# linuxing3/weekend-raytracer-wgpu

Measured on AMD Instinct MI355X. Metric: Msamples/sec (pixels x spp) at 1920x1080, 1000 spp, higher is better.
Workload: dtype f32; 1 GPU; BASELINE configs[2]: path-traced 3-sphere scene, checker-diffuse ground + glass + metal (src/main.rs:539-541), 1920x1080, 1000 spp, 8 bounces, gradient sky, seed 0; width=1920, height=1080, spp=1000, num_bounces=8, mode=pt, partition=whole frame

## Files before the change

include/mirt.h:

```cpp
#ifndef MIRT_H
#define MIRT_H

#include <stddef.h>
#include <stdint.h>

#ifdef __cplusplus
extern "C" {
#endif

#define MIRT_VERSION_MAJOR 0
#define MIRT_VERSION_MINOR 4
#define MIRT_VERSION_PATCH 0


typedef struct MirtSphere {
    float    center[4];
    float    radius;
    uint32_t material_idx;
    uint32_t _pad[2];
} MirtSphere;

typedef struct MirtTextureDescriptor {
    uint32_t width;
    uint32_t height;
// ... 134 lines not shown
typedef struct MirtContext MirtContext;


uint32_t    mirt_version(void);
const char* mirt_last_error(void);
const char* mirt_status_string(int status);

int mirt_validate_render_params(const MirtCamera* camera, const MirtSamplingParams* sampling,
                                uint32_t viewport_w, uint32_t viewport_h);

int mirt_camera_new(const MirtCamera* camera, uint32_t viewport_w, uint32_t viewport_h,
                    MirtGpuCamera* out);

int mirt_camera_from_fly_pose(const float position[3], float yaw_radians, float pitch_radians,
                              float vfov_degrees, float aperture, float focus_distance,
                              MirtCamera* out);

float mirt_degrees_to_radians(float degrees);
float mirt_radians_to_degrees(float radians);

uint32_t mirt_params_out_rows(const MirtParams* params);
uint32_t mirt_params_out_row_index(const MirtParams* params, uint32_t i);

typedef struct MirtGridPlan {
    float    cell_factor;
    uint32_t blob_bytes;
    uint32_t n_cells;
    uint32_t n_entries;
    uint32_t n_big;
    uint32_t pool_slots;
} MirtGridPlan;
int mirt_grid_plan(const MirtSphere* spheres, uint32_t n_spheres, uint64_t lds_bytes_per_block, MirtGridPlan* out);

int  mirt_ctx_create(int device, MirtContext** out);
void mirt_ctx_destroy(MirtContext* ctx);

int mirt_ctx_set_scene(MirtContext* ctx, const MirtScene* scene);
enum {
    MIRT_SCENE_HBM = 1u << 0
};
#define MIRT_SCENE_HBM_MAX_SPHERES (1u << 24)
#define MIRT_BVH_MAX_DEPTH  32
#define MIRT_BVH_MAX_LEAF   4
#define MIRT_BVH_MAX_ALWAYS 64
#define MIRT_BVH_BIG_RADII  4
int mirt_ctx_set_scene_ex(MirtContext* ctx, const MirtScene* scene, uint32_t flags);
typedef struct MirtBvhPlan {
    uint32_t n_nodes, n_leaves, n_leaf_spheres, n_always, max_depth, max_leaf;
    uint64_t device_bytes;
} MirtBvhPlan;
int mirt_bvh_plan(const MirtSphere* spheres, uint32_t n_spheres, MirtBvhPlan* out);

int mirt_ctx_set_camera(MirtContext* ctx, const MirtGpuCamera* camera);

int mirt_ctx_render(MirtContext* ctx, const MirtParams* params, uint8_t* out_rgba8, size_t out_len);

int mirt_ctx_render_device(MirtContext* ctx, const MirtParams* params, void* d_out_rgba8,
                           size_t out_len, void* hip_stream);

const char* mirt_ctx_last_kernel(const MirtContext* ctx);

int mirt_ctx_synchronize(MirtContext* ctx);
int mirt_ctx_frame_stream(MirtContext* ctx, uint32_t index, void** out_hip_stream);
int mirt_ctx_set_timing(MirtContext* ctx, int enabled);
int mirt_ctx_get_stats(MirtContext* ctx, MirtStats* out);

// ... 73 lines not shown
```

rust/mirt-sys/src/lib.rs:

```rust
#![allow(non_camel_case_types)]

use std::os::raw::{c_char, c_int, c_void};

#[repr(C)]
#[derive(Clone, Copy, Debug, Default)]
pub struct MirtSphere {
    pub center: [f32; 4],
    pub radius: f32,
    pub material_idx: u32,
    pub _pad: [u32; 2],
}

#[repr(C)]
#[derive(Clone, Copy, Debug, Default)]
pub struct MirtTextureDescriptor {
    pub width: u32,
    pub height: u32,
    pub offset: u32,
}

#[repr(C)]
#[derive(Clone, Copy, Debug, Default)]
pub struct MirtMaterial {
    pub id: u32,
// ... 171 lines not shown
pub struct MirtContext {
    _private: [u8; 0],
}

pub const MIRT_NODE_MAX_MEMBERS: u32 = 16;
pub const MIRT_NODE_RCCL: u32 = 1 << 0;

#[repr(C)]
pub struct MirtNode {
    _private: [u8; 0],
}

#[repr(C)]
#[derive(Clone, Copy, Debug, Default)]
pub struct MirtNodeStats {
    pub n_members: u32,
    pub transport: u32,
    pub gather_ms: f64,
    pub assemble_ms: f64,
}

extern "C" {
    pub fn mirt_version() -> u32;
    pub fn mirt_last_error() -> *const c_char;
    pub fn mirt_status_string(status: c_int) -> *const c_char;
    pub fn mirt_validate_render_params(camera: *const MirtCamera, sampling: *const MirtSamplingParams, viewport_w: u32, viewport_h: u32) -> c_int;
    pub fn mirt_camera_new(camera: *const MirtCamera, viewport_w: u32, viewport_h: u32, out: *mut MirtGpuCamera) -> c_int;
    pub fn mirt_camera_from_fly_pose(position: *const f32, yaw_radians: f32, pitch_radians: f32, vfov_degrees: f32, aperture: f32, focus_distance: f32, out: *mut MirtCamera) -> c_int;
    pub fn mirt_degrees_to_radians(degrees: f32) -> f32;
    pub fn mirt_radians_to_degrees(radians: f32) -> f32;
    pub fn mirt_params_out_rows(params: *const MirtParams) -> u32;
    pub fn mirt_params_out_row_index(params: *const MirtParams, i: u32) -> u32;
    pub fn mirt_grid_plan(spheres: *const MirtSphere, n_spheres: u32, lds_bytes_per_block: u64, out: *mut MirtGridPlan) -> c_int;
    pub fn mirt_ctx_create(device: c_int, out: *mut *mut MirtContext) -> c_int;
    pub fn mirt_ctx_destroy(ctx: *mut MirtContext);
    pub fn mirt_ctx_set_scene(ctx: *mut MirtContext, scene: *const MirtScene) -> c_int;
    pub fn mirt_ctx_set_scene_ex(ctx: *mut MirtContext, scene: *const MirtScene, flags: u32) -> c_int;
    pub fn mirt_bvh_plan(spheres: *const MirtSphere, n_spheres: u32, out: *mut MirtBvhPlan) -> c_int;
    pub fn mirt_ctx_set_camera(ctx: *mut MirtContext, camera: *const MirtGpuCamera) -> c_int;
    pub fn mirt_ctx_render(ctx: *mut MirtContext, params: *const MirtParams, out_rgba8: *mut u8, out_len: usize) -> c_int;
    pub fn mirt_ctx_render_device(ctx: *mut MirtContext, params: *const MirtParams, d_out_rgba8: *mut c_void, out_len: usize, hip_stream: *mut c_void) -> c_int;
    pub fn mirt_ctx_synchronize(ctx: *mut MirtContext) -> c_int;
    pub fn mirt_ctx_get_stats(ctx: *mut MirtContext, out: *mut MirtStats) -> c_int;
    pub fn mirt_ctx_frame_stream(ctx: *mut MirtContext, index: u32, out_hip_stream: *mut *mut c_void) -> c_int;
    pub fn mirt_ctx_set_timing(ctx: *mut MirtContext, enabled: c_int) -> c_int;
    pub fn mirt_ctx_last_kernel(ctx: *const MirtContext) -> *const c_char;
    pub fn mirt_ctx_accum_reset(ctx: *mut MirtContext, params: *const MirtParams) -> c_int;
    pub fn mirt_ctx_accum_add(ctx: *mut MirtContext, params: *const MirtParams, hip_stream: *mut c_void) -> c_int;
    pub fn mirt_ctx_accum_samples(ctx: *const MirtContext) -> u32;
    pub fn mirt_ctx_accum_resolve(ctx: *mut MirtContext, params: *const MirtParams, out_rgba8: *mut u8, out_len: usize) -> c_int;
    pub fn mirt_ctx_accum_read(ctx: *mut MirtContext, out_sums: *mut u64, out_len_u64: usize) -> c_int;
    pub fn mirt_ctx_accum_frame_device(ctx: *mut MirtContext, params: *const MirtParams, d_out_rgba8: *mut c_void, out_len: usize, hip_stream: *mut c_void) -> c_int;
    pub fn mirt_ctx_accum_frame(ctx: *mut MirtContext, params: *const MirtParams, out_rgba8: *mut u8, out_len: usize) -> c_int;
    pub fn mirt_ctx_selftest_math(ctx: *mut MirtContext, out_mismatches: *mut u64) -> c_int;
    pub fn mirt_render(scene: *const MirtScene, params: *const MirtParams, device: c_int, out_rgba8: *mut u8, out_len: usize) -> c_int;
    pub fn mirt_rgba8_to_rgb8(rgba: *const u8, n_pixels: usize, rgb: *mut u8) -> c_int;
    pub fn mirt_jpeg_info(data: *const u8, len: usize, width: *mut u32, height: *mut u32) -> c_int;
    pub fn mirt_jpeg_decode_rgb8(data: *const u8, len: usize, rgb: *mut u8, rgb_len: usize) -> c_int;
    pub fn mirt_rgb8_to_texels(rgb: *const u8, n_pixels: usize, texels: *mut f32) -> c_int;
    pub fn mirt_jpeg_last_error() -> *const c_char;
    pub fn mirt_ctx_deinterleave_device(ctx: *mut MirtContext, params: *const MirtParams, d_parts: *const c_void, part_stride: usize, d_out_rgba8: *mut c_void, out_len: usize, hip_stream: *mut c_void) -> c_int;
    pub fn mirt_node_create(devices: *const c_int, n: u32, flags: u32, out: *mut *mut MirtNode) -> c_int;
    pub fn mirt_node_destroy(node: *mut MirtNode);
    pub fn mirt_node_set_scene(node: *mut MirtNode, scene: *const MirtScene) -> c_int;
    pub fn mirt_node_set_scene_ex(node: *mut MirtNode, scene: *const MirtScene, flags: u32) -> c_int;
    pub fn mirt_node_set_camera(node: *mut MirtNode, camera: *const MirtGpuCamera) -> c_int;
// ... 11 lines not shown
```

weekend-raytracer-wgpu_amd/_abi.py:

```python
from __future__ import annotations

import ctypes as C

MIRT_MODE_PARITY = 0
MIRT_MODE_PT = 1
MIRT_MAX_SPP_PER_CALL = 1 << 24

MIRT_FLAG_SKY_HOSEK = 1 << 0
MIRT_FLAG_NO_TONEMAP = 1 << 1
MIRT_FLAG_NO_SRGB = 1 << 2
MIRT_FLAG_COUNT_WORK = 1 << 3
MIRT_FLAG_KERNEL_STRIP = 1 << 4
MIRT_FLAG_KERNEL_POOL = 1 << 5
MIRT_FLAG_NO_GRID = 1 << 6
MIRT_FLAG_COUNT_GRID = 1 << 7
MIRT_FLAG_FAST_MATH = 1 << 8
MIRT_FLAG_TEXEL_TILES = 1 << 9

MIRT_SCENE_HBM = 1 << 0
MIRT_SCENE_HBM_MAX_SPHERES = 1 << 24
MIRT_BVH_MAX_DEPTH = 32
MIRT_BVH_MAX_LEAF = 4
MIRT_BVH_MAX_ALWAYS = 64
MIRT_BVH_BIG_RADII = 4
# ... 108 lines not shown

    def as_dict(self) -> dict:
        return {"kernel_ms": self.kernel_ms, "kernel_ms_total": self.kernel_ms_total, "launches": self.launches,
                "samples": self.samples, "rays": self.rays,
                "sphere_tests": self.sphere_tests, "roots": self.roots, "hits": self.hits,
                "scatter": list(self.scatter), "sky_misses": self.sky_misses,
                "lane_iterations": self.lane_iterations, "wave_iterations": self.wave_iterations,
                "grid_cells": self.grid_cells, "grid_wave_cells": self.grid_wave_cells,
                "texel_fetches": list(self.texel_fetches), "texel_tile_hits": list(self.texel_tile_hits)}


class MirtNodeStats(C.Structure):
    _fields_ = [("n_members", C.c_uint32), ("transport", C.c_uint32), ("gather_ms", C.c_double), ("assemble_ms", C.c_double)]

    def as_dict(self) -> dict:
        return {"n_members": self.n_members, "transport": self.transport, "gather_ms": self.gather_ms,
                "assemble_ms": self.assemble_ms}


_P = C.POINTER
SYMBOLS = {
    "mirt_version": (C.c_uint32, []),
    "mirt_last_error": (C.c_char_p, []),
    "mirt_status_string": (C.c_char_p, [C.c_int]),
    "mirt_validate_render_params": (C.c_int, [_P(MirtCamera), _P(MirtSamplingParams), C.c_uint32, C.c_uint32]),
    "mirt_camera_new": (C.c_int, [_P(MirtCamera), C.c_uint32, C.c_uint32, _P(MirtGpuCamera)]),
    "mirt_camera_from_fly_pose": (C.c_int, [_P(C.c_float), C.c_float, C.c_float, C.c_float, C.c_float,
                                            C.c_float, _P(MirtCamera)]),
    "mirt_degrees_to_radians": (C.c_float, [C.c_float]),
    "mirt_radians_to_degrees": (C.c_float, [C.c_float]),
    "mirt_params_out_rows": (C.c_uint32, [_P(MirtParams)]),
    "mirt_params_out_row_index": (C.c_uint32, [_P(MirtParams), C.c_uint32]),
    "mirt_grid_plan": (C.c_int, [C.c_void_p, C.c_uint32, C.c_uint64, _P(MirtGridPlan)]),
    "mirt_ctx_create": (C.c_int, [C.c_int, _P(C.c_void_p)]),
    "mirt_ctx_destroy": (None, [C.c_void_p]),
    "mirt_ctx_set_scene": (C.c_int, [C.c_void_p, _P(MirtScene)]),
    "mirt_ctx_set_scene_ex": (C.c_int, [C.c_void_p, _P(MirtScene), C.c_uint32]),
    "mirt_bvh_plan": (C.c_int, [C.c_void_p, C.c_uint32, _P(MirtBvhPlan)]),
    "mirt_ctx_set_camera": (C.c_int, [C.c_void_p, _P(MirtGpuCamera)]),
    "mirt_ctx_render": (C.c_int, [C.c_void_p, _P(MirtParams), C.c_void_p, C.c_size_t]),
    "mirt_ctx_render_device": (C.c_int, [C.c_void_p, _P(MirtParams), C.c_void_p, C.c_size_t, C.c_void_p]),
    "mirt_ctx_last_kernel": (C.c_char_p, [C.c_void_p]),
    "mirt_ctx_synchronize": (C.c_int, [C.c_void_p]),
    "mirt_ctx_get_stats": (C.c_int, [C.c_void_p, _P(MirtStats)]),
    "mirt_ctx_accum_reset": (C.c_int, [C.c_void_p, _P(MirtParams)]),
    "mirt_ctx_accum_add": (C.c_int, [C.c_void_p, _P(MirtParams), C.c_void_p]),
    "mirt_ctx_accum_samples": (C.c_uint32, [C.c_void_p]),
    "mirt_ctx_accum_resolve": (C.c_int, [C.c_void_p, _P(MirtParams), C.c_void_p, C.c_size_t]),
    "mirt_ctx_accum_read": (C.c_int, [C.c_void_p, C.c_void_p, C.c_size_t]),
    "mirt_ctx_accum_frame_device": (C.c_int, [C.c_void_p, _P(MirtParams), C.c_void_p, C.c_size_t, C.c_void_p]),
    "mirt_ctx_accum_frame": (C.c_int, [C.c_void_p, _P(MirtParams), C.c_void_p, C.c_size_t]),
    "mirt_ctx_selftest_math": (C.c_int, [C.c_void_p, _P(C.c_uint64)]),
    "mirt_ctx_set_timing": (C.c_int, [C.c_void_p, C.c_int]),
    "mirt_ctx_frame_stream": (C.c_int, [C.c_void_p, C.c_uint32, C.POINTER(C.c_void_p)]),
    "mirt_render": (C.c_int, [_P(MirtScene), _P(MirtParams), C.c_int, C.c_void_p, C.c_size_t]),
    "mirt_rgba8_to_rgb8": (C.c_int, [C.c_void_p, C.c_size_t, C.c_void_p]),
    "mirt_jpeg_info": (C.c_int, [C.c_void_p, C.c_size_t, _P(C.c_uint32), _P(C.c_uint32)]),
    "mirt_jpeg_decode_rgb8": (C.c_int, [C.c_void_p, C.c_size_t, C.c_void_p, C.c_size_t]),
    "mirt_rgb8_to_texels": (C.c_int, [C.c_void_p, C.c_size_t, C.c_void_p]),
    "mirt_jpeg_last_error": (C.c_char_p, []),
    "mirt_ctx_deinterleave_device": (C.c_int, [C.c_void_p, _P(MirtParams), C.c_void_p, C.c_size_t,
                                               C.c_void_p, C.c_size_t, C.c_void_p]),
    "mirt_node_create": (C.c_int, [_P(C.c_int), C.c_uint32, C.c_uint32, _P(C.c_void_p)]),
    "mirt_node_destroy": (None, [C.c_void_p]),
    "mirt_node_set_scene": (C.c_int, [C.c_void_p, _P(MirtScene)]),
    "mirt_node_set_scene_ex": (C.c_int, [C.c_void_p, _P(MirtScene), C.c_uint32]),
# ... 19 lines not shown
```

weekend-raytracer-wgpu_amd/csrc/mirt_api.hip:

```cpp
#include <hip/hip_runtime.h>

#include <algorithm>
#include <cmath>
#include <cstdarg>
#include <cstdio>
#include <cstdlib>
#include <cstring>
#include <new>
#include <vector>

#include "../../include/mirt.h"
#include "mirt_kernels.h"
#include "mirt_bvh.h"

namespace kx = mirt::exact_build;
namespace kf = mirt::fast_build;

namespace {

thread_local char g_err[512] = "";

int fail(int status, const char* fmt, ...)
{
    va_list ap;
// ... 162 lines not shown
std::vector<unsigned char> plan_grid(const MirtSphere* sph, uint32_t n, double cell_knob, double big_knob, size_t lds_per_block, double* factor_out)
{
    std::vector<unsigned char> grid;
    double f = cell_knob > 0.0 ? cell_knob : 2.5;
    for (;; f = std::min(f * 1.26, 4.0)) {
        bool overflow = false;
        grid = build_grid(sph, n, f, big_knob, &overflow);
        if (cell_knob > 0.0 || f >= 4.0) break;
        if (grid.empty()) { if (overflow) continue; break; }
        const size_t beside = kx::scene_lds_bytes_grid(n, true) + grid.size();
        if (beside < lds_per_block && kx::pool_config_grid(lds_per_block - beside).slots >= 152u) break;
    }
    if (factor_out) *factor_out = grid.empty() ? 0.0 : f;
    return grid;
}

struct Tuning {
    int      pool_config = -1;
    int      pool_grid = -1;
    bool     fixed_strips = false;
    uint32_t gss_min_width = 0;
    double   gss_keep = 0.0;
    int      by_pixel = -1;
    uint32_t pool_blocks_per_cu = 0;
    double   grid_cell = 0.0;
    double   grid_big = 0.0;
    int      pinhole = -1;
    int      spread_units = -1;
    int      static_units = -1;
    int      pool_min_spp = -1;
    int      stream = -1;
    int      px_groups = -1;
    int      strip_cand = -1;
    int      grid_flat_y = -1;
    bool     debug_slots = false;
    uint32_t static_block = 0;
    int      static_grid = -1;
    int      timing = -1;
    bool     ext_events = true;
};

Tuning read_tuning()
{
    Tuning t;
    if (const char* e = std::getenv("MIRT_POOL_CONFIG")) { const long v = std::strtol(e, nullptr, 10); if (v >= 0 && (uint32_t)v < kx::pool_config_count()) t.pool_config = (int)v; }
    if (const char* e = std::getenv("MIRT_POOL_GRID")) t.pool_grid = (e[0] == '0') ? 0 : 1;
    if (const char* e = std::getenv("MIRT_STRIP_MODE")) t.fixed_strips = e[0] == '1';
    if (const char* e = std::getenv("MIRT_GSS_MINW")) { const uint32_t v = (uint32_t)std::atoi(e); if (v >= 1 && v <= 16) t.gss_min_width = v; }
    if (const char* e = std::getenv("MIRT_GSS_KEEP")) { const double v = std::atof(e); if (v > 0.0 && v < 64.0) t.gss_keep = v; }
    if (const char* e = std::getenv("MIRT_BY_PIXEL")) t.by_pixel = (e[0] == '1') ? 1 : 0;
    if (const char* e = std::getenv("MIRT_POOL_BLOCKS_PER_CU")) { const uint32_t v = (uint32_t)std::atoi(e); if (v >= 1) t.pool_blocks_per_cu = v; }
    if (const char* e = std::getenv("MIRT_GRID_CELL")) { const double v = std::atof(e); if (v >= 1.0 && v <= 64.0) t.grid_cell = v; }
    if (const char* e = std::getenv("MIRT_PINHOLE")) t.pinhole = (e[0] == '0') ? 0 : 1;
    if (const char* e = std::getenv("MIRT_SPREAD_UNITS")) t.spread_units = (e[0] == '0') ? 0 : 1;
    if (const char* e = std::getenv("MIRT_STATIC_UNITS")) t.static_units = (e[0] == '1') ? 1 : 0;
    if (const char* e = std::getenv("MIRT_POOL_MIN_SPP")) { const int v = std::atoi(e); if (v >= 1) t.pool_min_spp = v; }
    if (const char* e = std::getenv("MIRT_STREAM")) t.stream = std::atoi(e) != 0 ? 1 : 0;
    if (const char* e = std::getenv("MIRT_PX_GROUPS")) { const int v = std::atoi(e); if (v >= 0 && v <= 3) t.px_groups = v; }
    if (const char* e = std::getenv("MIRT_STRIP_CAND")) t.strip_cand = (e[0] == '0') ? 0 : 1;
    if (const char* e = std::getenv("MIRT_GRID_FLAT_Y")) t.grid_flat_y = (e[0] == '0') ? 0 : 1;
    if (const char* e = std::getenv("MIRT_DEBUG_SLOTS")) t.debug_slots = e[0] == '1';
    if (const char* e = std::getenv("MIRT_STATIC_BLOCK")) { const int v = std::atoi(e); if (v == 64 || v == 128 || v == 256) t.static_block = (uint32_t)v; }
    if (const char* e = std::getenv("MIRT_STATIC_GRID")) { const int v = std::atoi(e); if (v >= 1 && v <= 64) t.static_grid = v; }
    if (const char* e = std::getenv("MIRT_TIMING")) t.timing = (e[0] == '0') ? 0 : 1;
    if (const char* e = std::getenv("MIRT_EXT_EVENTS")) t.ext_events = e[0] != '0';
    if (const char* e = std::getenv("MIRT_GRID_BIG")) { const double v = std::atof(e); if (v >= 1.0 && v <= 1024.0) t.grid_big = v; }
    return t;
}

bool camera_is_pinhole(const MirtGpuCamera& cam)
{
    if (cam.lens_radius != 0.0f) return false;
    for (int k = 0; k < 3; ++k) {
        if (!std::isfinite(cam.u[k]) || !std::isfinite(cam.v[k]) || !std::isfinite(cam.eye[k])) return false;
        if (cam.eye[k] == 0.0f && std::signbit(cam.eye[k])) return false;
    }
    return true;
}

template <typename T>
int ensure_capacity(T** ptr, size_t* cap, size_t need)
{
    if (need <= *cap && *ptr) return MIRT_OK;
    if (*ptr) (void)hipFree(*ptr);
    *ptr = nullptr;
    *cap = 0;
    const size_t bytes = (need ? need : 1) * sizeof(T);
    if (hipMalloc(ptr, bytes) != hipSuccess) return fail(MIRT_ERR_ALLOC, "hipMalloc(%zu bytes) failed", bytes);
    *cap = need ? need : 1;
    return MIRT_OK;
}

// ... 184 lines not shown
    out->aperture = aperture;
    out->focus_distance = focus_distance;
    return MIRT_OK;
}

uint32_t mirt_params_out_rows(const MirtParams* params) { return out_rows(params); }

uint32_t mirt_params_out_row_index(const MirtParams* p, uint32_t i)
{
    uint32_t rb, re;
    if (!p || !rows_valid(p, &rb, &re) || i >= out_rows(p)) return UINT32_MAX;
    if (p->tile_rows == 0 || p->n_parts <= 1) return rb + i;
    const uint32_t t = p->part + (i / p->tile_rows) * p->n_parts;
    return rb + t * p->tile_rows + i % p->tile_rows;
}

int mirt_grid_plan(const MirtSphere* spheres, uint32_t n_spheres, uint64_t lds_bytes_per_block, MirtGridPlan* out)
{
    if (!out || (n_spheres && !spheres)) return fail(MIRT_ERR_NULL_POINTER, "spheres/out is null");
    *out = MirtGridPlan{};
    const size_t lds = lds_bytes_per_block ? (size_t)lds_bytes_per_block : (size_t)160 * 1024;
    double f = 0.0;
    const Tuning tune = read_tuning();
    const std::vector<unsigned char> grid = plan_grid(spheres, n_spheres, tune.grid_cell, tune.grid_big, lds, &f);
    if (grid.empty() || n_spheres > 4095u || kx::scene_lds_bytes_grid(n_spheres, true) + grid.size() > mirt::kMaxLdsBytes) return MIRT_OK;
    const mirt::GridHeader* gh = reinterpret_cast<const mirt::GridHeader*>(grid.data());
    out->cell_factor = (float)f;
    out->blob_bytes = (uint32_t)grid.size();
    out->n_cells = gh->dims[0] * gh->dims[1] * gh->dims[2];
    out->n_entries = gh->n_entries;
    out->n_big = gh->n_big;
    const size_t beside = kx::scene_lds_bytes_grid(n_spheres, true) + grid.size();
    out->pool_slots = beside < lds ? kx::pool_config_grid(lds - beside).slots : 0u;
    return MIRT_OK;
}

int mirt_ctx_create(int device, MirtContext** out)
{
    if (!out) return fail(MIRT_ERR_NULL_POINTER, "out is null");
    *out = nullptr;
    int n = 0;
    if (hipGetDeviceCount(&n) != hipSuccess || n <= 0)
        return fail(MIRT_ERR_NO_DEVICE, "no HIP device visible (this library has no CPU fallback)");
    if (device < 0 || device >= n) return fail(MIRT_ERR_NO_DEVICE, "device %d out of range (0..%d)", device, n - 1);
    MirtContext* c = new (std::nothrow) MirtContext();
    if (!c) return fail(MIRT_ERR_ALLOC, "out of host memory");
    c->device = device;
    hipDeviceProp_t prop;
    hipError_t e = hipSetDevice(device);
    if (e == hipSuccess) e = hipGetDeviceProperties(&prop, device);
    if (e == hipSuccess) e = hipStreamCreateWithFlags(&c->stream, hipStreamNonBlocking);
    for (int i = 0; i < kEventPool && e == hipSuccess; ++i) {
        hipEvent_t a = nullptr, b = nullptr;
        e = hipEventCreate(&a);
        if (e == hipSuccess) e = hipEventCreate(&b);
        if (a) c->ev_begin.push_back(a);
        if (b) c->ev_end.push_back(b);
        hipEvent_t z = nullptr;
        if (e == hipSuccess) e = hipEventCreateWithFlags(&z, hipEventDisableTiming);
        if (z) c->ev_zeroed.push_back(z);
    }
    c->slot_busy.assign(kEventPool, 0);
    c->slot_zeroing.assign(kEventPool, 0);
    c->slot_dirty.assign(kEventPool, 0);
    c->slot_zero_event.assign(kEventPool, 0);
    c->slot_timed.assign(kEventPool, 0);
// ... 404 lines not shown
        const uint64_t waves = (uint64_t)c->cu_count * (resident_pool_waves < 32u ? resident_pool_waves : 32u);
        uint32_t min_width = 4;
        while (min_width < mirt::kStripPixels && (uint64_t)min_width * p->spp < 512u) min_width *= 2;
        if (tune.fixed_strips) min_width = mirt::kStripPixels;
        if (tune.gss_min_width) min_width = tune.gss_min_width;
        const double keep_factor = tune.gss_keep > 0.0 ? tune.gss_keep : 4.0;
        uint64_t pix = 0, unit = 0;
        for (uint32_t l = 0; l < mirt::kStripLevels; ++l) {
            const uint32_t width = mirt::kStripPixels >> l;
            a.lvl_unit[l] = (uint32_t)unit;
            a.lvl_pix[l] = (uint32_t)pix;
            uint64_t level_px;
            if (width <= min_width) {
                level_px = npix - pix;
            } else {
                const uint64_t keep = (uint64_t)(keep_factor * (double)(waves * width));
                const uint64_t left = npix - pix;
                level_px = left > keep ? (left - keep) / width * width : 0;
            }
            pix += level_px;
            unit += (level_px + width - 1) / width;
        }
        a.lvl_unit[mirt::kStripLevels] = (uint32_t)unit;
        a.lvl_pix[mirt::kStripLevels] = (uint32_t)npix;
        a.n_units = (uint32_t)unit;
    }
    const bool use_grid = pool_grid || (grid_ok && !pool && scene_lds_g + c->grid_bytes + 4u * 48u <= (size_t)c->lds_per_block);
    a.grid = use_grid ? c->d_grid : nullptr;
    a.grid_bytes = use_grid ? c->grid_bytes : 0u;
    a.shade = (use_grid && c->have_shade) ? c->d_shade : nullptr;
    a.grid_pool_slots = pool_grid ? pcg.slots : 0u;
    a.strip_cand = (use_grid && tune.strip_cand != 0 && (pool_grid || p->spp >= 4u)) ? 1u : 0u;
    a.grid_flat_y = (use_grid && c->grid_flat_y) ? 1u : 0u;
    a.lds_bytes = use_grid ? (uint32_t)(scene_lds_g + a.grid_bytes + (pool ? pcu.lds_bytes : 4u * 48u)) : (uint32_t)(scene_lds + (pool ? pcu.lds_bytes : 0));
    const bool hbm = c->hbm;
    const bool hbm_bvh = hbm && pt && !(p->flags & MIRT_FLAG_NO_GRID) && (!count || (p->flags & MIRT_FLAG_COUNT_GRID));
    if (hbm) {
        a.bvh_nodes = reinterpret_cast<const float4*>(c->d_bvh);
        a.bvh_recs = reinterpret_cast<const float4*>(c->d_bvh + c->bvh_off_recs);
        a.bvh_ids = reinterpret_cast<const uint32_t*>(c->d_bvh + c->bvh_off_ids);
        a.bvh_root = c->bvh_root;
        a.bvh_n_always = c->bvh_n_always;
        for (int k = 0; k < 3; ++k) a.bvh_centre[k] = c->bvh_centre[k];
        a.bvh_radius = c->bvh_radius;
        a.bvh_rmax = c->bvh_rmax;
    }
    if (!use_grid && !c->fits_flat && !hbm)
        return fail(MIRT_ERR_SCENE_TOO_LARGE, "this scene only fits LDS in the grid build of the path-traced mode "
                    "(no parity mode, no MIRT_FLAG_COUNT_WORK / MIRT_FLAG_NO_GRID / MIRT_FLAG_KERNEL_POOL)");

    bool by_pixel = pt && !pool && !count && (p->spp < mirt::kByPixelMaxSpp || (c->n_shading_routines <= 1 && npix >= 64ull * 4u * c->cu_count));
    if (tune.by_pixel >= 0) by_pixel = pt && !pool && !count && tune.by_pixel == 1;
    if (hbm_bvh && !count) by_pixel = true;
    if (frame_stream) by_pixel = true;
    if (!pt) by_pixel = (p->flags & MIRT_FLAG_KERNEL_STRIP) ? false : (tune.by_pixel >= 0 ? tune.by_pixel == 1 : true);
    a.static_units = 0;
    a.px_groups_log2 = 0;
    a.stream_samples = (pt && by_pixel && !count && !use_grid && p->spp >= 16u) ? 1u : 0u;
    if (tune.stream >= 0 && pt && by_pixel && !count && !use_grid) a.stream_samples = (uint32_t)tune.stream;
    if (hbm) a.stream_samples = 0u;
    if (by_pixel) {
        if (pt && !frame_stream && tune.px_groups != 0) {
            const uint32_t min_share[2] = { a.stream_samples ? 8u : 4u, a.stream_samples ? 8u : (use_grid ? 4u : 6u) };
            while (a.px_groups_log2 < 2u && p->spp % (2u << a.px_groups_log2) == 0u && (p->spp >> (a.px_groups_log2 + 1u)) >= min_share[a.px_groups_log2])
                a.px_groups_log2 += 1u;
            if (tune.px_groups > 0 && p->spp % (1u << (tune.px_groups - 1)) == 0u) a.px_groups_log2 = (uint32_t)tune.px_groups - 1u;
// ... 448 lines not shown
```

weekend-raytracer-wgpu_amd/csrc/mirt_kernels.h:

```cpp
#pragma once

#include <hip/hip_runtime.h>
#include <stdint.h>

#include "../../include/mirt.h"

namespace mirt {

struct PreparedSphere {
    float    cx, cy, cz, rr;
    float    inv_r, radius;
    uint32_t material_idx;
    uint32_t op;
};
static_assert(sizeof(PreparedSphere) == 32, "PreparedSphere must stay 2 x 16 B for ds_read_b128");

struct PreparedMaterial {
    uint32_t id;
    float    x;
    float    inv_x;
    uint32_t flags;
    float    tex[2][4];
};
static_assert(sizeof(PreparedMaterial) == 48, "PreparedMaterial is 3 x 16 B");

struct ShadeRec {
    float a[4];
    float t0[4];
    float t1[4];
    float c[4];
};
static_assert(sizeof(ShadeRec) == 64, "ShadeRec is one 64-byte line");

struct GridHeader {
    float    org[3];
    float    cell[3];
    float    inv_cell[3];
    uint32_t dims[3];
// ... 70 lines not shown
    uint32_t                grid_bytes;
    uint32_t                grid_pool_slots;
    uint32_t                strip_cand;
    uint32_t                grid_flat_y;
    uint32_t*               work_counter;
    unsigned long long*     accum;
    uint64_t                n_texels;
    uint32_t n_spheres, n_mats;
    uint32_t width, height, spp, num_bounces, flags, seed_mix, sample_begin;
    uint32_t frame_begin;
    uint32_t frame_spp;
    uint32_t row_begin, tile_rows, n_parts, part;
    uint32_t out_rows;
    uint32_t n_units;
    uint32_t first_dispensed;
    uint32_t disp_taken[8];
    uint32_t static_units;
    uint32_t spread_units;
    uint32_t px_groups_log2;
    uint32_t lvl_unit[6];
    uint32_t lvl_pix[6];
    uint32_t queue_routine[5];
    uint32_t lds_bytes;
    uint32_t launch_threads;
    uint32_t stream_samples;
    float    sph3[12];
    const float4*   bvh_nodes;
    const float4*   bvh_recs;
    const uint32_t* bvh_ids;
    uint32_t        bvh_root;
    uint32_t        bvh_n_always;
    float           bvh_centre[3];
    float           bvh_radius, bvh_rmax;
};
constexpr uint32_t kBvhStackBytesPerWave = 64u * MIRT_BVH_MAX_DEPTH * 4u;

constexpr uint32_t kAssembleMaxParts = 16;
struct AssembleArgs {
    const uint32_t* parts[kAssembleMaxParts];
    uint32_t*       out;
    uint64_t        part_stride_px;
    uint32_t        width, band_rows, tile_rows, n_parts;
    uint32_t        vec4;
};

struct LaunchOn {
    hipStream_t stream = nullptr;
    hipEvent_t  begin = nullptr, end = nullptr;
    LaunchOn(hipStream_t s = nullptr, hipEvent_t b = nullptr, hipEvent_t e = nullptr) : stream(s), begin(b), end(e) {}
};

struct PoolConfig { uint32_t threads, slots, lds_bytes; };
namespace fast_build {
hipError_t launch_pt_strip(const RenderArgs& a, uint32_t grid_blocks, bool count, bool use_grid, bool by_pixel, LaunchOn stream);
uint32_t   strip_blocks_per_cu(bool hosek, bool count, bool use_grid, bool by_pixel, uint32_t lds_bytes, bool stream, bool frame = false);
hipError_t launch_pt_pool(const RenderArgs& a, uint32_t grid_blocks, uint32_t cfg, bool count, uint32_t nq, LaunchOn stream);
hipError_t launch_pt_hbm(const RenderArgs& a, uint32_t grid_blocks, bool count, bool bvh, bool by_pixel, LaunchOn stream);
uint32_t   hbm_blocks_per_cu(bool hosek, bool count, bool bvh, bool by_pixel, uint32_t threads, uint32_t lds_bytes, bool frame = false);
}
namespace exact_build {
hipError_t launch_pt_hbm(const RenderArgs& a, uint32_t grid_blocks, bool count, bool bvh, bool by_pixel, LaunchOn stream);
uint32_t   hbm_blocks_per_cu(bool hosek, bool count, bool bvh, bool by_pixel, uint32_t threads, uint32_t lds_bytes, bool frame = false);
hipError_t launch_parity_hbm(const RenderArgs& a, uint32_t grid_blocks, bool count, bool by_pixel, LaunchOn stream);
uint32_t   parity_hbm_blocks_per_cu(bool count, bool by_pixel, uint32_t threads, uint32_t lds_bytes);
hipError_t launch_parity(const RenderArgs& a, uint32_t grid_blocks, bool count, bool by_pixel, LaunchOn stream);
hipError_t launch_pt_strip(const RenderArgs& a, uint32_t grid_blocks, bool count, bool use_grid, bool by_pixel, LaunchOn stream);
// ... 21 lines not shown
```

weekend-raytracer-wgpu_amd/csrc/mirt_kernels.hip:

```cpp
#include <cstdio>
#include <mutex>

#include <hip/hip_ext.h>
#include "mirt_kernels.h"
#include "mirt_device_math.h"
#include "mirt_device_resolve.h"

namespace mirt {
namespace MIRT_KNS {


struct SceneLds {
    const float*            cam;
    const PreparedSphere*   spheres;
    const MirtMaterial*     mats;
    const PreparedMaterial* pmats;
    const float*            sky;
    unsigned char*          end;
};

template <bool PT, bool MATS_IN_LDS = true>
MIRT_DEV SceneLds stage_scene(const RenderArgs& A, unsigned char* smem, bool hosek)
{
    constexpr uint32_t kMatQuads = PT ? sizeof(PreparedMaterial) / 16 : sizeof(MirtMaterial) / 16;
// ... 1602 lines not shown

template <bool COUNT, bool HOSEK, bool BVH, bool BY_PIXEL>
__global__ __launch_bounds__(kBlockThreads, (BY_PIXEL && !COUNT) ? 6 : 1) void render_pt_hbm_frame_kernel(RenderArgs A)
{
    strip_kernel_body<COUNT, HOSEK, false, BY_PIXEL, false, BVH ? kSrcBvh : kSrcHbmFlat, true>(A);
}

template <bool HOSEK>
__global__ __launch_bounds__(kBlockThreads, HOSEK ? 6 : 8) void render_pt_stream_frame_kernel(RenderArgs A)
{
    strip_kernel_body<false, HOSEK, false, true, true, kSrcLds, true>(A);
}

constexpr uint32_t RT_LAMBERTIAN = 0, RT_METAL = 1, RT_DIELECTRIC = 2, RT_CHECKER = 3;
constexpr uint32_t OP_NONE = 7, kMaxQueues = 6;
#ifndef MIRT_FF_MIN
#define MIRT_FF_MIN 64
#endif
constexpr uint32_t kFastForwardMin = MIRT_FF_MIN;

template <uint32_t SLOTS, uint32_t NQ, bool GRID = false, bool TILE = false>
struct WavePoolLayout {
    static constexpr uint32_t kQueues   = NQ + 1 + (GRID ? 1 : 0);
    static constexpr uint32_t kRing     = SLOTS;
    static constexpr uint32_t kOffState = 0;
    static constexpr uint32_t kOffAcc   = kOffState + SLOTS * 48;
    static constexpr uint32_t kOffCell  = kOffAcc + kStripPixels * 3 * 8;
    static constexpr uint32_t kOffRing  = kOffCell + (GRID ? SLOTS * 2 : 0);
    static constexpr uint32_t kOffCand  = ((kOffRing + kQueues * kRing + 15) / 16) * 16;
    static constexpr uint32_t kOffTile  = kOffCand + (GRID ? kCandBytes : 0);
    static constexpr uint32_t kBytes    = kOffTile + (TILE ? ((kTileBytes + 15) / 16) * 16 : 0);
};

#define MIRT_POOL_KERNEL_FRAME false
#define MIRT_POOL_KERNEL_NAME render_pt_pool_kernel
#define MIRT_POOL_KERNEL_TILE false
#include "mirt_pool_kernel.inc"
#undef MIRT_POOL_KERNEL_NAME
#undef MIRT_POOL_KERNEL_TILE
#define MIRT_POOL_KERNEL_NAME render_pt_pool_tile_kernel
#define MIRT_POOL_KERNEL_TILE true
#include "mirt_pool_kernel.inc"
#undef MIRT_POOL_KERNEL_NAME
#undef MIRT_POOL_KERNEL_TILE
#undef MIRT_POOL_KERNEL_FRAME
#define MIRT_POOL_KERNEL_FRAME true
#define MIRT_POOL_KERNEL_NAME render_pt_pool_frame_kernel
#define MIRT_POOL_KERNEL_TILE false
#include "mirt_pool_kernel.inc"
#undef MIRT_POOL_KERNEL_NAME
#undef MIRT_POOL_KERNEL_TILE
#define MIRT_POOL_KERNEL_NAME render_pt_pool_tile_frame_kernel
#define MIRT_POOL_KERNEL_TILE true
#include "mirt_pool_kernel.inc"
#undef MIRT_POOL_KERNEL_NAME
#undef MIRT_POOL_KERNEL_TILE
#undef MIRT_POOL_KERNEL_FRAME

#ifdef MIRT_ISA_PROBES
#include "mirt_isa_probes.inc"
#endif

#ifndef MIRT_FAST_MATH

__global__ __launch_bounds__(256) void selftest_math_kernel(unsigned long long* mismatches)
{
// ... 424 lines not shown
```

weekend-raytracer-wgpu_amd/csrc/mirt_pool_kernel.inc:

```
template <uint32_t THREADS, uint32_t SLOTS, uint32_t MINW, bool COUNT, bool HOSEK, uint32_t NQ = 5, bool GRID = false, bool FLATY = false>
__global__ __launch_bounds__(THREADS, MINW) void MIRT_POOL_KERNEL_NAME(RenderArgs A)
{
    constexpr bool TILE = MIRT_POOL_KERNEL_TILE;
    constexpr bool FRAME = MIRT_POOL_KERNEL_FRAME;
    using Lay = WavePoolLayout<SLOTS, NQ, GRID, TILE>;
    static_assert(!(GRID && TILE), "the tile build exists for flat scenes");
    static_assert(GRID || !FLATY, "FLATY: a grid one cell high");
    constexpr uint32_t OP_GEN = NQ, OP_WALK = NQ + 1, kNumOps = Lay::kQueues;
    static_assert(NQ >= 1 && NQ < kMaxQueues, "scatter queues");
    constexpr uint32_t RING = Lay::kRing;
    static_assert(SLOTS >= 64 && SLOTS <= 256 && SLOTS % 8 == 0, "slot ids are 8 bit");
    extern __shared__ __align__(16) unsigned char smem[];
    const SceneLds S = stage_scene<true, !GRID>(A, smem, HOSEK);
    const uint32_t tid = threadIdx.x;
    const uint32_t lane = tid & 63u;
    const uint32_t wave = __builtin_amdgcn_readfirstlane(tid >> 6);
    uint32_t scene_bytes = (uint32_t)scene_lds_bytes_dev(A.n_spheres, A.n_mats, HOSEK, !GRID);
    GridLds G{};
    if constexpr (GRID) { G = stage_grid(A, smem + scene_bytes); scene_bytes += A.grid_bytes; }
    constexpr bool HOLD_CAM = !GRID && !HOSEK && !TILE && !COUNT && MINW == 6;
    CamHeld CH{};
    if constexpr (HOLD_CAM) CH = hold_camera(S);
    GridConsts GC{};
    if constexpr (GRID) GC = load_grid_consts(G);
    unsigned char* pool = smem + scene_bytes + wave * Lay::kBytes;
    uint4* const L_state = reinterpret_cast<uint4*>(pool + Lay::kOffState);
    unsigned long long* const L_acc = reinterpret_cast<unsigned long long*>(pool + Lay::kOffAcc);
    unsigned char* const L_ring = pool + Lay::kOffRing;
    unsigned short* const L_cell = reinterpret_cast<unsigned short*>(pool + Lay::kOffCell);
    unsigned short* const L_cand = reinterpret_cast<unsigned short*>(pool + Lay::kOffCand);
    uint32_t* const L_cand_n = reinterpret_cast<uint32_t*>(pool + Lay::kOffCand + 2 * kMaxCand);
    TexelTile tile{ reinterpret_cast<uint32_t*>(pool + Lay::kOffTile), reinterpret_cast<float*>(pool + Lay::kOffTile + 16), 0u, 0u, 0u, 0u, 0u, 0u };
    TexelTile* const T = TILE ? &tile : nullptr;

    Work<COUNT> work;
    work.clear();
    Stamps stamps;
    stamps.start();

    for (uint32_t strip = first_unit(); strip < A.n_units; strip = next_unit_any(A, lane)) {
        const RenderArgs& AP = per_strip_args();
        uint32_t lvl = 0;
#pragma unroll
        for (uint32_t l = 1; l < kStripLevels; ++l) lvl = (strip >= AP.lvl_unit[l]) ? l : lvl;
        uint32_t unit0 = AP.lvl_unit[0], pix0 = AP.lvl_pix[0], pix_end = AP.lvl_pix[1];
#pragma unroll
        for (uint32_t l = 1; l < kStripLevels; ++l)
            if (lvl == l) { unit0 = AP.lvl_unit[l]; pix0 = AP.lvl_pix[l]; pix_end = AP.lvl_pix[l + 1]; }
        const uint32_t width_log2 = 4u - lvl;
        const uint32_t base_pix = pix0 + ((strip - unit0) << width_log2);
        const uint32_t want_pixels = 1u << width_log2;
        const uint32_t strip_pixels = (pix_end - base_pix < want_pixels) ? (pix_end - base_pix) : want_pixels;
        const uint32_t total_items = strip_pixels * AP.spp;
        const uint32_t base_ci = base_pix / AP.width;
        const uint32_t base_x = base_pix - base_ci * AP.width;
        const bool wide = AP.width >= kStripPixels;
        const uint32_t row0 = abs_row(AP, base_ci);
        const uint32_t row1 = (base_ci + 1 < AP.out_rows) ? abs_row(AP, base_ci + 1) : row0;

        for (uint32_t s = lane; s < SLOTS; s += 64) { L_ring[OP_GEN * RING + s] = (unsigned char)s; L_state[s * 3].w = 0u; }
        if (lane < kStripPixels * 3) L_acc[lane] = 0ull;
        if constexpr (TILE) tile.reset(lane);
        if constexpr (GRID) {
            uint32_t n_cand = kNoCand;
            if (AP.strip_cand != 0u && wide && base_x + strip_pixels <= AP.width)
                n_cand = strip_candidates(AP, S, base_x, strip_pixels, row0, L_cand, lane);
            if (lane == 0) *L_cand_n = n_cand;
#define MIRT_PROBE_SITE 6
#include "mirt_pool_probes.inc"
#undef MIRT_PROBE_SITE
        }
        uint32_t tail[kNumOps];
#pragma unroll
        for (uint32_t k = 0; k < kNumOps; ++k) tail[k] = (k == OP_GEN) ? SLOTS : 0u;
        uint32_t next_item = 0;

        bool ff = false;
        uint32_t my_k = 0, my_n = 0;
        uint32_t slot = 0, pix = 0, bounce = 0, missf = 0;
        int best = 0;
        float walk_closest = kMaxT;
        uint32_t walk_cell = 0;
        f3 ro = mk(0, 0, 0), rd = mk(0, 0, 0), thr = mk(0, 0, 0);
        Rng rng;
        rng.state = 0;

        for (;;) {
            stamps.mark(6);
            if (!ff) {
                uint32_t key = 0;
#pragma unroll
                for (uint32_t k = 0; k < kNumOps; ++k) {
                    const uint32_t kk = (tail[k] << 3) | (7u - k);
                    key = (kk > key) ? kk : key;
                }
// ... 226 lines not shown
```

Baseline: 89650 Msamples/s.

## Shade strips whose primary-ray cone misses every sphere directly from the sky

Adds a conservative per-strip visibility test that bounds the primary-ray cone (including lens aperture) against each sphere. When no sphere can be hit, the pool kernel skips the wavefront queue machinery and accumulates sky colour for all samples directly. This avoids the path-tracing pipeline for pure-sky strips, at the cost of a per-strip cone test and a dependence on the test being conservative enough to keep the image identical.

After: 90990 Msamples/s, median of 6. 1.5% higher.

```diff
diff --git a/include/mirt.h b/include/mirt.h
--- a/include/mirt.h
+++ b/include/mirt.h
@@ -190,6 +190,9 @@
 } MirtGridPlan;
 int mirt_grid_plan(const MirtSphere* spheres, uint32_t n_spheres, uint64_t lds_bytes_per_block, MirtGridPlan* out);
 
+int mirt_strip_visibility(const MirtSphere* spheres, uint32_t n_spheres, const MirtGpuCamera* camera, uint32_t width, uint32_t height,
+                          uint32_t x0, uint32_t n_pixels, uint32_t row, uint32_t* mask);
+
 int  mirt_ctx_create(int device, MirtContext** out);
 void mirt_ctx_destroy(MirtContext* ctx);
 
diff --git a/rust/mirt-sys/src/lib.rs b/rust/mirt-sys/src/lib.rs
--- a/rust/mirt-sys/src/lib.rs
+++ b/rust/mirt-sys/src/lib.rs
@@ -227,6 +227,7 @@
     pub fn mirt_params_out_rows(params: *const MirtParams) -> u32;
     pub fn mirt_params_out_row_index(params: *const MirtParams, i: u32) -> u32;
     pub fn mirt_grid_plan(spheres: *const MirtSphere, n_spheres: u32, lds_bytes_per_block: u64, out: *mut MirtGridPlan) -> c_int;
+    pub fn mirt_strip_visibility(spheres: *const MirtSphere, n_spheres: u32, camera: *const MirtGpuCamera, width: u32, height: u32, x0: u32, n_pixels: u32, row: u32, mask: *mut u32) -> c_int;
     pub fn mirt_ctx_create(device: c_int, out: *mut *mut MirtContext) -> c_int;
     pub fn mirt_ctx_destroy(ctx: *mut MirtContext);
     pub fn mirt_ctx_set_scene(ctx: *mut MirtContext, scene: *const MirtScene) -> c_int;
diff --git a/weekend-raytracer-wgpu_amd/_abi.py b/weekend-raytracer-wgpu_amd/_abi.py
--- a/weekend-raytracer-wgpu_amd/_abi.py
+++ b/weekend-raytracer-wgpu_amd/_abi.py
@@ -164,6 +164,8 @@
     "mirt_params_out_rows": (C.c_uint32, [_P(MirtParams)]),
     "mirt_params_out_row_index": (C.c_uint32, [_P(MirtParams), C.c_uint32]),
     "mirt_grid_plan": (C.c_int, [C.c_void_p, C.c_uint32, C.c_uint64, _P(MirtGridPlan)]),
+    "mirt_strip_visibility": (C.c_int, [C.c_void_p, C.c_uint32, _P(MirtGpuCamera), C.c_uint32, C.c_uint32, C.c_uint32, C.c_uint32, C.c_uint32,
+                                        _P(C.c_uint32)]),
     "mirt_ctx_create": (C.c_int, [C.c_int, _P(C.c_void_p)]),
     "mirt_ctx_destroy": (None, [C.c_void_p]),
     "mirt_ctx_set_scene": (C.c_int, [C.c_void_p, _P(MirtScene)]),
diff --git a/weekend-raytracer-wgpu_amd/csrc/mirt_api.hip b/weekend-raytracer-wgpu_amd/csrc/mirt_api.hip
--- a/weekend-raytracer-wgpu_amd/csrc/mirt_api.hip
+++ b/weekend-raytracer-wgpu_amd/csrc/mirt_api.hip
@@ -218,6 +218,7 @@
     int      stream = -1;
     int      px_groups = -1;
     int      strip_cand = -1;
+    int      strip_vis = -1;
     int      grid_flat_y = -1;
     bool     debug_slots = false;
     uint32_t static_block = 0;
@@ -244,6 +245,7 @@
     if (const char* e = std::getenv("MIRT_STREAM")) t.stream = std::atoi(e) != 0 ? 1 : 0;
     if (const char* e = std::getenv("MIRT_PX_GROUPS")) { const int v = std::atoi(e); if (v >= 0 && v <= 3) t.px_groups = v; }
     if (const char* e = std::getenv("MIRT_STRIP_CAND")) t.strip_cand = (e[0] == '0') ? 0 : 1;
+    if (const char* e = std::getenv("MIRT_STRIP_VIS")) t.strip_vis = (e[0] == '0') ? 0 : 1;
     if (const char* e = std::getenv("MIRT_GRID_FLAT_Y")) t.grid_flat_y = (e[0] == '0') ? 0 : 1;
     if (const char* e = std::getenv("MIRT_DEBUG_SLOTS")) t.debug_slots = e[0] == '1';
     if (const char* e = std::getenv("MIRT_STATIC_BLOCK")) { const int v = std::atoi(e); if (v == 64 || v == 128 || v == 256) t.static_block = (uint32_t)v; }
@@ -494,6 +496,17 @@
     out->n_big = gh->n_big;
     const size_t beside = kx::scene_lds_bytes_grid(n_spheres, true) + grid.size();
     out->pool_slots = beside < lds ? kx::pool_config_grid(lds - beside).slots : 0u;
+    return MIRT_OK;
+}
+
+int mirt_strip_visibility(const MirtSphere* spheres, uint32_t n_spheres, const MirtGpuCamera* camera, uint32_t width, uint32_t height,
+                          uint32_t x0, uint32_t n_pixels, uint32_t row, uint32_t* mask)
+{
+    if (!mask || !camera || (n_spheres && !spheres)) return fail(MIRT_ERR_NULL_POINTER, "spheres/camera/mask is null");
+    static_assert(sizeof(MirtSphere) == 32 && offsetof(MirtSphere, radius) == 16, "strip_visibility reads 8-float records, radius in [4]");
+    const uint32_t m = mirt::strip_visibility(reinterpret_cast<const float*>(camera), reinterpret_cast<const float*>(spheres), 4u, n_spheres,
+                                              width, height, x0, n_pixels, row);
+    *mask = (m == mirt::kVisNone) ? 0u : m;
     return MIRT_OK;
 }
 
@@ -964,6 +977,8 @@
     a.grid_pool_slots = pool_grid ? pcg.slots : 0u;
     a.strip_cand = (use_grid && tune.strip_cand != 0 && (pool_grid || p->spp >= 4u)) ? 1u : 0u;
     a.grid_flat_y = (use_grid && c->grid_flat_y) ? 1u : 0u;
+    a.strip_vis = (pool && !use_grid && !count && !hosek && !tiles && tune.strip_vis != 0 && c->n_spheres <= mirt::kVisMax &&
+                   p->num_bounces >= 1u && !(p->flags & MIRT_FLAG_FAST_MATH)) ? 1u : 0u;
     a.lds_bytes = use_grid ? (uint32_t)(scene_lds_g + a.grid_bytes + (pool ? pcu.lds_bytes : 4u * 48u)) : (uint32_t)(scene_lds + (pool ? pcu.lds_bytes : 0));
     const bool hbm = c->hbm;
     const bool hbm_bvh = hbm && pt && !(p->flags & MIRT_FLAG_NO_GRID) && (!count || (p->flags & MIRT_FLAG_COUNT_GRID));
diff --git a/weekend-raytracer-wgpu_amd/csrc/mirt_kernels.h b/weekend-raytracer-wgpu_amd/csrc/mirt_kernels.h
--- a/weekend-raytracer-wgpu_amd/csrc/mirt_kernels.h
+++ b/weekend-raytracer-wgpu_amd/csrc/mirt_kernels.h
@@ -4,6 +4,7 @@
 #include <stdint.h>
 
 #include "../../include/mirt.h"
+#include "mirt_strip_vis.h"
 
 namespace mirt {
 
@@ -140,6 +141,7 @@
     uint32_t        bvh_n_always;
     float           bvh_centre[3];
     float           bvh_radius, bvh_rmax;
+    uint32_t        strip_vis;
 };
 constexpr uint32_t kBvhStackBytesPerWave = 64u * MIRT_BVH_MAX_DEPTH * 4u;
 
diff --git a/weekend-raytracer-wgpu_amd/csrc/mirt_kernels.hip b/weekend-raytracer-wgpu_amd/csrc/mirt_kernels.hip
--- a/weekend-raytracer-wgpu_amd/csrc/mirt_kernels.hip
+++ b/weekend-raytracer-wgpu_amd/csrc/mirt_kernels.hip
@@ -1658,6 +1658,37 @@
     static constexpr uint32_t kBytes    = kOffTile + (TILE ? ((kTileBytes + 15) / 16) * 16 : 0);
 };
 
+MIRT_DEV void sky_strip(const RenderArgs& A, const SceneLds& S, const CamRegs& C, uint32_t base_x, uint32_t y, uint32_t strip_pixels,
+                        uint32_t want_pixels, uint32_t width_log2, uint32_t total_items, uint32_t lane, unsigned long long* L_acc)
+{
+    const bool full = strip_pixels == want_pixels;
+    unsigned long long sr = 0ull, sg = 0ull, sb = 0ull;
+    uint32_t pix = lane & (want_pixels - 1u);
+    for (uint32_t item0 = 0; item0 < total_items; item0 += 64u) {
+        const uint32_t item = item0 + lane;
+        uint32_t sample;
+        if (full) sample = item >> width_log2;
+        else { sample = item / strip_pixels; pix = item - sample * strip_pixels; }
+        Rng rng;
+        f3 ro, rd;
+        generate_primary(A, C, base_x + pix, y, A.sample_begin + sample, rng, ro, rd);
+        const f3 c = sky_color<false>(S, rd);
+        if (item < total_items) {
+            if (full) { sr += to_fixed(c.x); sg += to_fixed(c.y); sb += to_fixed(c.z); }
+            else {
+                atomicAdd(&L_acc[pix * 3 + 0], (unsigned long long)to_fixed(c.x));
+                atomicAdd(&L_acc[pix * 3 + 1], (unsigned long long)to_fixed(c.y));
+                atomicAdd(&L_acc[pix * 3 + 2], (unsigned long long)to_fixed(c.z));
+            }
+        }
+    }
+    if (full) {
+        atomicAdd(&L_acc[pix * 3 + 0], sr);
+        atomicAdd(&L_acc[pix * 3 + 1], sg);
+        atomicAdd(&L_acc[pix * 3 + 2], sb);
+    }
+}
+
 #define MIRT_POOL_KERNEL_FRAME false
 #define MIRT_POOL_KERNEL_NAME render_pt_pool_kernel
 #define MIRT_POOL_KERNEL_TILE false
diff --git a/weekend-raytracer-wgpu_amd/csrc/mirt_pool_kernel.inc b/weekend-raytracer-wgpu_amd/csrc/mirt_pool_kernel.inc
--- a/weekend-raytracer-wgpu_amd/csrc/mirt_pool_kernel.inc
+++ b/weekend-raytracer-wgpu_amd/csrc/mirt_pool_kernel.inc
@@ -51,7 +51,7 @@
         const uint32_t base_pix = pix0 + ((strip - unit0) << width_log2);
         const uint32_t want_pixels = 1u << width_log2;
         const uint32_t strip_pixels = (pix_end - base_pix < want_pixels) ? (pix_end - base_pix) : want_pixels;
-        const uint32_t total_items = strip_pixels * AP.spp;
+        uint32_t total_items = strip_pixels * AP.spp;
         const uint32_t base_ci = base_pix / AP.width;
         const uint32_t base_x = base_pix - base_ci * AP.width;
         const bool wide = AP.width >= kStripPixels;
@@ -61,6 +61,16 @@
         for (uint32_t s = lane; s < SLOTS; s += 64) { L_ring[OP_GEN * RING + s] = (unsigned char)s; L_state[s * 3].w = 0u; }
         if (lane < kStripPixels * 3) L_acc[lane] = 0ull;
         if constexpr (TILE) tile.reset(lane);
+        if constexpr (!GRID && !COUNT && !TILE && !HOSEK) {
+            if (AP.strip_vis != 0u && wide) {
+                const uint32_t vis = __builtin_amdgcn_readfirstlane(strip_visibility(S.cam, reinterpret_cast<const float*>(S.spheres), 5u, AP.n_spheres,
+                                                                                      AP.width, AP.height, base_x, strip_pixels, row0));
+                if (vis == (1u << AP.n_spheres) - 1u) {
+                    sky_strip(A, S, load_camera(S, A), base_x, row0, strip_pixels, want_pixels, width_log2, total_items, lane, L_acc);
+                    total_items = 0u;
+                }
+            }
+        }
         if constexpr (GRID) {
             uint32_t n_cand = kNoCand;
             if (AP.strip_cand != 0u && wide && base_x + strip_pixels <= AP.width)
diff --git a/weekend-raytracer-wgpu_amd/csrc/mirt_strip_vis.h b/weekend-raytracer-wgpu_amd/csrc/mirt_strip_vis.h
--- /dev/null
+++ b/weekend-raytracer-wgpu_amd/csrc/mirt_strip_vis.h
@@ -0,0 +1,72 @@
+#pragma once
+
+#include <stdint.h>
+
+#if defined(__HIPCC__) || defined(__CUDACC__)
+#define MIRT_VIS_FN __host__ __device__ inline
+#else
+#define MIRT_VIS_FN inline
+#endif
+
+namespace mirt {
+
+constexpr uint32_t kVisMax = 8;
+constexpr uint32_t kVisNone = 0x80000000u;
+
+MIRT_VIS_FN uint32_t strip_visibility(const float* cam, const float* sph, uint32_t radius_at, uint32_t n_spheres,
+                                      uint32_t width, uint32_t height, uint32_t x0, uint32_t n, uint32_t y)
+{
+    if (n_spheres > kVisMax || n == 0u || n > 16u || width < 16u || height == 0u || x0 + n > width || y >= height) return kVisNone;
+    const float ex = cam[0], ey = cam[1], ez = cam[2];
+    const float hx = cam[4], hy = cam[5], hz = cam[6];
+    const float vx = cam[8], vy = cam[9], vz = cam[10];
+    const float ux = cam[12], uy = cam[13], uz = cam[14];
+    const float wx = cam[16], wy = cam[17], wz = cam[18];
+    const float lens_radius = cam[19];
+    const float lx = cam[20], ly = cam[21], lz = cam[22];
+    const float inv_w = 1.0f / (float)width, inv_h = 1.0f / (float)height;
+    const float u0 = (float)x0 * inv_w, u1 = (float)(x0 + n) * inv_w;
+    const float v1 = 1.0f - (float)y * inv_h, v0 = 1.0f - (float)(y + 1u) * inv_h;
+    const float uc = 0.5f * (u0 + u1), vc = 0.5f * (v0 + v1), du = 0.5f * (u1 - u0), dv = 0.5f * (v1 - v0);
+    const float ax = (lx + uc * hx + vc * vx) - ex, ay = (ly + uc * hy + vc * vy) - ey, az = (lz + uc * hz + vc * vz) - ez;
+    const float D = __builtin_sqrtf(ax * ax + ay * ay + az * az);
+    const float len_h = __builtin_sqrtf(hx * hx + hy * hy + hz * hz), len_v = __builtin_sqrtf(vx * vx + vy * vy + vz * vz);
+    const float len_l = __builtin_sqrtf(lx * lx + ly * ly + lz * lz), len_e = __builtin_sqrtf(ex * ex + ey * ey + ez * ez);
+    const float delta = __builtin_fabsf(du) * len_h + __builtin_fabsf(dv) * len_v + 1.0e-6f * (len_h + len_v + len_l + len_e);
+    const float uu = ux * ux + uy * uy + uz * uz, ww = wx * wx + wy * wy + wz * wz, uw = ux * wx + uy * wy + uz * wz;
+    const float hd = 0.5f * (uu - ww);
+    const float lambda = 0.5f * (uu + ww) + __builtin_sqrtf(hd * hd + uw * uw);
+    const float R = 1.03f * __builtin_fabsf(lens_radius) * __builtin_sqrtf(lambda);
+    const float g = 1.02f * (delta + R) + 1.0e-6f * D;
+    if (!(D > 0.0f && D < 1.0e30f && g < 0.25f * D)) return kVisNone;
+    const float inv_D = 1.0f / D;
+    const float hx_ = inv_D * ax, hy_ = inv_D * ay, hz_ = inv_D * az;
+    const float dl = 1.02f * delta + 1.0e-6f * D;
+    const float beta0 = dl - R, beta1 = dl + R;
+    const float k0 = beta0 / __builtin_sqrtf(D * D - beta0 * beta0), k1 = beta1 / __builtin_sqrtf(D * D - beta1 * beta1);
+    uint32_t mask = 0u;
+    for (uint32_t i = 0; i < n_spheres; ++i) {
+        const float* sp = sph + 8u * i;
+        const float qx = sp[0] - ex, qy = sp[1] - ey, qz = sp[2] - ez;
+        const float r = __builtin_fabsf(sp[radius_at]);
+        const float len_q = __builtin_sqrtf(qx * qx + qy * qy + qz * qz);
+        const float cx = qy * hz_ - qz * hy_, cy = qz * hx_ - qx * hz_, cz = qx * hy_ - qy * hx_;
+        const float dperp = __builtin_sqrtf(cx * cx + cy * cy + cz * cz);
+        const float L = len_q + r + R;
+        const float qa = qx * ax + qy * ay + qz * az;
+        const float t0 = (qa * inv_D) * inv_D;
+        float ta = t0 + k0 * dperp * inv_D, tb = t0 + k1 * dperp * inv_D;
+        ta = ta > 0.0f ? (ta < 1.0f ? ta : 1.0f) : 0.0f;
+        tb = tb > 1.0f ? tb : 1.0f;
+        const float wa = D * (ta - t0), wb = D * (tb - t0);
+        const float ha = __builtin_sqrtf(wa * wa + dperp * dperp) - (R + beta0 * ta);
+        const float hb = __builtin_sqrtf(wb * wb + dperp * dperp) - (beta1 * tb - R);
+        const float dmin = (ha < hb ? ha : hb) - 1.0e-5f * L;
+        const bool clear = (dmin > r) && ((dmin - r) * (dmin + r) > 0x1p-14f * (L * L));
+        const bool away = (-qa > len_q * g + R * (D + g) + 1.0e-4f * (len_q + R) * (D + g)) && (len_q > r + R + 1.0e-5f * L);
+        if (clear || away) mask |= 1u << i;
+    }
+    return mask;
+}
+
+}
```
